# esw0116/DynaVSR

Hardware: AMD Instinct MI355X
Metric: inner-loop frames/sec/GPU (EDVR-M x4, 5x3x180x320): forward leg = BASELINE.json configs[1]; the inner MAML step and the per-frame pipeline are `inner_step` / `per_frame_pipeline` (higher is better)
Workload: dtype f32; 1 GPU; EDVR-M x4 forward (PCD deformable alignment + TSA fusion + reconstruction), clips of 1x5x3x180x320 -> 3x720x1280 (BASELINE.json configs[1]); one step = 2 clip(s) per GPU, one per HIP stream (adapt.super_resolve_video); clips_in_flight_per_gpu=2

## Files before the change

### dynavsr_amd/_lib.py

```python
import ctypes
import os
from ctypes import POINTER, Structure, c_char_p, c_float, c_int, c_longlong, c_size_t, c_void_p

import torch

_runtime = {"configured": False, "hw_queues": None, "effective": None}


def configure_runtime(hw_queues=6):
    if not _runtime["configured"]:
        user = os.environ.get("GPU_MAX_HW_QUEUES")
        late = torch.cuda.is_initialized()
        if user is None and not late:
            os.environ["GPU_MAX_HW_QUEUES"] = str(int(hw_queues))
        _runtime.update(configured=True, hw_queues=os.environ.get("GPU_MAX_HW_QUEUES"),
                        effective=(user is not None) or not late)
    return {"hw_queues": _runtime["hw_queues"], "effective": _runtime["effective"]}


def runtime_report(device=None):
    r = configure_runtime()
    overlaps = None
    if torch.cuda.is_available():
        with torch.cuda.device(device if device is not None else torch.cuda.current_device()):
# ... 81 lines not shown
        "dvsr_adam_step": (I, [POINTER(c_void_p)] * 4 + [POINTER(LL), I, F, F, F, F, F, I, P]),
        "dvsr_sgd_step": (I, [POINTER(c_void_p)] * 2 + [POINTER(LL), I, F, F, P]),
        "dvsr_replicate_tensors": (I, [POINTER(c_void_p)] * 2 + [POINTER(LL), I, I, P]),
        "dvsr_degrade_apply": (I, [P, P, P, I, I, I, I, I, I, I, I, I, P]),
        "dvsr_frame_metrics_workspace_bytes": (c_size_t, [I, I, I]),
        "dvsr_frame_metrics": (I, [P, P, I, I, I, F, F, P, P, P, c_size_t, P]),
        "dvsr_charbonnier_workspace_bytes": (c_size_t, []),
        "dvsr_charbonnier_forward": (I, [P, P, P, LL, F, P, c_size_t, P]),
        "dvsr_conv2d_packed_workspace_bytes": (c_size_t, [POINTER(Conv2dDesc)]),
        "dvsr_conv2d_forward_packed": (I, [POINTER(Conv2dDesc), P, c_size_t, P]),
        "dvsr_conv2d_dgrad_packed": (I, [POINTER(Conv2dDesc), P, P, P, c_size_t, P]),
        "dvsr_conv2d_packed_geometry": (I, [POINTER(Conv2dDesc), POINTER(ctypes.c_int * 4)]),
        "dvsr_conv2d_wgrad_geometry": (I, [POINTER(Conv2dDesc), I, I, POINTER(ctypes.c_int * 8)]),
        "dvsr_conv2d_wgrad_workspace_bytes": (c_size_t, [POINTER(Conv2dDesc), I]),
        "dvsr_conv2d_wgrad_bf16": (I, [POINTER(Conv2dDesc), P, P, P, P, c_size_t, P]),
        "dvsr_conv2d_wgrad_split3": (I, [POINTER(Conv2dDesc), P, P, P, P, c_size_t, P]),
        "dvsr_flow_warp_forward": (I, [P, P, P, I, I, I, I, LL, P]),
        "dvsr_flow_warp_backward": (I, [P, P, P, P, P, I, I, I, I, LL, P]),
        "dvsr_avgpool2_forward": (I, [P, P, LL, I, I, P]),
        "dvsr_avgpool2_backward": (I, [P, P, LL, I, I, I, P]),
        "dvsr_resize_bilinear_ac_forward": (I, [P, P, LL, I, I, I, I, F, LL, P]),
        "dvsr_resize_bilinear_ac_backward": (I, [P, P, LL, I, I, I, I, F, LL, P]),
        "dvsr_upsample_bicubic_ac_forward": (I, [P, P, LL, I, I, I, P]),
        "dvsr_upsample_bicubic_ac_backward": (I, [P, P, LL, I, I, I, P]),
        "dvsr_channel_affine": (I, [P, P, P, P, I, I, LL, LL, LL, I, P]),
        "dvsr_batchnorm_workspace_bytes": (c_size_t, [I]),
        "dvsr_batchnorm_forward": (I, [P] * 8 + [I, I, LL, I, F, F, I, P, c_size_t, P]),
        "dvsr_batchnorm_backward": (I, [P] * 9 + [I, I, LL, I, I, P, c_size_t, P]),
        "dvsr_temporal_gather3_forward": (I, [P, P, I, I, I, LL, I, P]),
        "dvsr_temporal_gather3_backward": (I, [P, P, I, I, I, LL, I, P]),
        "dvsr_dynamic_filter_forward": (I, [P, P, P, P, I, I, I, I, I, P]),
        "dvsr_dynamic_filter_backward": (I, [P, P, P, P, P, P, I, I, I, I, I, P]),
        "dvsr_conv3x3_small_cout": (I, [P, P, P, P, P, I, I, I, I, I, I, P]),
        "dvsr_conv1x1_dual": (I, [P, P, P, P, P, P, P, I, I, I, I, I, P]),
        "dvsr_patch_gather_forward": (I, [P, P, POINTER(c_int), POINTER(c_int), I, I, I, I, I, I, P]),
        "dvsr_patch_gather_backward": (I, [P, P, POINTER(c_int), POINTER(c_int), I, I, I, I, I, I, P]),
        "dvsr_l1_tail_forward": (I, [P, P, P, F, P, LL, P, c_size_t, P]),
        "dvsr_l1_tail_backward": (I, [P, P, P, F, P, LL, P]),
        "dvsr_charbonnier_backward": (I, [P, P, P, P, LL, F, P]),
        "dvsr_charbonnier_forward_grouped": (I, [P, P, P, LL, I, F, P, c_size_t, P]),
        "dvsr_charbonnier_backward_grouped": (I, [P, P, P, P, LL, I, F, P]),
        "dvsr_l1_tail_forward_grouped": (I, [P, P, P, F, P, LL, I, P, c_size_t, P]),
        "dvsr_l1_tail_backward_grouped": (I, [P, P, P, F, P, LL, I, P]),
        "dvsr_edvr_op_info": (I, [P, I, c_char_p, I, c_char_p, I, POINTER(ctypes.c_double),
                                  POINTER(ctypes.c_double)]),
        "dvsr_edvr_forward_timed": (I, [P, POINTER(c_void_p), P, P, P, c_size_t, P, POINTER(c_float)]),
        "dvsr_debug_mfma_peak": (LL, [P, I, I, I, I, P]),
        "dvsr_debug_mfma_shadow": (I, [P, P, I, I, I, I, I, P]),
        "dvsr_edvr_tensor_info": (I, [P, c_char_p, POINTER(LL), POINTER(LL)]),
        "dvsr_edvr_plan_work": (I, [P, POINTER(ctypes.c_double * 9)]),
        "dvsr_edvr_plan_work_nograd": (I, [P, POINTER(ctypes.c_double * 9)]),
        "dvsr_edvr_op_launch_count": (I, [P, I, I]),
        "dvsr_side_stream_overlaps": (I, [P]),
        "dvsr_edvr_op_output": (I, [P, I, I, POINTER(c_int), POINTER(LL), POINTER(LL)]),
        "dvsr_estimator_plan_work": (I, [P, POINTER(ctypes.c_double * 9)]),
        "dvsr_edvr_stream_create": (I, [POINTER(EdvrConfig), I, I, I, POINTER(c_void_p)]),
        "dvsr_edvr_stream_destroy": (None, [P]),
        "dvsr_edvr_stream_num_params": (I, [P]),
        "dvsr_edvr_stream_num_launches": (I, [P, I]),
        "dvsr_edvr_stream_cache_bytes": (c_size_t, [P]),
        "dvsr_edvr_stream_workspace_bytes": (c_size_t, [P]),
        "dvsr_edvr_stream_extract": (I, [P, POINTER(c_void_p), P, I, P, c_size_t, P, c_size_t, I, P]),
        "dvsr_edvr_stream_fuse": (I, [P, POINTER(c_void_p), POINTER(c_int), P, c_size_t, P, P, c_size_t, I, P]),
        "dvsr_frame_ingest": (I, [P, POINTER(FrameDesc), P, I, I, I, P]),
        "dvsr_frame_emit": (I, [P, I, I, P, POINTER(FrameDesc), F, F, P]),
        "dvsr_edvr_stream_extract_frame": (I, [P, POINTER(c_void_p), P, POINTER(FrameDesc), I, I, P, c_size_t, P, c_size_t, I,
# ... 42 lines not shown
```

### dynavsr_amd/csrc/conv_small.hip

```cpp
#include "common.h"
#include "kernels.h"

namespace dvsr {

struct SmallK {
  const float* x; const float* w; const float* bias; const float* res; float* y;
  int N, C, H, W, Cout, act, tiles_x, tiles_y, ntiles;
  int wdiv; long long w_gs; int b_gs;
};

typedef float f32x2 __attribute__((ext_vector_type(2)));

template <int COUT>
__global__ __launch_bounds__(256) void conv3x3_small_cout_kernel(SmallK a) {
  constexpr int CC = 8, TH = 8, TW = 64, IH = TH + 2, IW = TW + 2, PLANE = IH * IW, E = (PLANE + 255) / 256;
  constexpr int WPC = ((9 * COUT + 3) / 4) * 4;
  __shared__ __attribute__((aligned(16))) float s_in[2][CC * PLANE];
  extern __shared__ __attribute__((aligned(16))) float s_w[];
  const int tpx = (a.ntiles + 7) >> 3;
  const int tile = (blockIdx.x & 7) * tpx + (blockIdx.x >> 3);
  if ((int)(blockIdx.x >> 3) >= tpx || tile >= a.ntiles) return;
  const int tx_ = tile % a.tiles_x;
  const int t2 = tile / a.tiles_x;
  const int ty_ = t2 % a.tiles_y;
  const int n = t2 / a.tiles_y;
  const int oy0 = ty_ * TH, ox0 = tx_ * TW;
  const int tid = threadIdx.x;
  const int py = tid >> 5, px2 = (tid & 31) * 2;
  const size_t HW = (size_t)a.H * a.W;
  const float* xn = a.x + (size_t)n * a.C * HW;
  const float* wn = wset_ptr(a.w, a.w_gs, n, a.wdiv);
  const float* bn = wset_ptr(a.bias, a.b_gs, n, a.wdiv);

  unsigned eoff[E];
  bool evalid[E];
#pragma unroll
  for (int e = 0; e < E; ++e) {
    const int idx = tid + 256 * e;
    const int iy = idx / IW, ix = idx - iy * IW;
    const int gy = oy0 - 1 + iy, gx = ox0 - 1 + ix;
// ... 51 lines not shown
            const float wv = wq[wi >> 2][wi & 3];
            acc[o] = __builtin_elementwise_fma(f32x2{wv, wv}, f32x2{v[tx], v[tx + 1]}, acc[o]);
          }
      }
    }
  }
  const int oy = oy0 + py, ox = ox0 + px2;
  if (oy >= a.H || ox >= a.W) return;
  const bool two = ox + 1 < a.W;
  float bvs[COUT];
  f32x2 rvs[COUT];
#pragma unroll
  for (int o = 0; o < COUT; ++o) {
    bvs[o] = bn ? bn[o] : 0.f;
    const size_t idx = ((size_t)n * a.Cout + o) * HW + (size_t)oy * a.W + ox;
    rvs[o] = (a.res && two && (idx & 1) == 0) ? *reinterpret_cast<const f32x2*>(a.res + idx) : f32x2{0.f, 0.f};
  }
#pragma unroll
  for (int o = 0; o < COUT; ++o) {
    const float bv = bvs[o];
    f32x2 v = {apply_act(acc[o][0] + bv, a.act), apply_act(acc[o][1] + bv, a.act)};
    const size_t idx = ((size_t)n * a.Cout + o) * HW + (size_t)oy * a.W + ox;
    if (two && (idx & 1) == 0) {
      v += rvs[o];
      *reinterpret_cast<f32x2*>(a.y + idx) = v;
    } else {
      a.y[idx] = v[0] + (a.res ? a.res[idx] : 0.f);
      if (two) a.y[idx + 1] = v[1] + (a.res ? a.res[idx + 1] : 0.f);
    }
  }
}

struct SmallMfmaShape {
  static constexpr int TH = 6, TW = 56, RH = 8, RW = 64, X0 = 4, NPOS = RH * RW, APITCH = 68;
  static constexpr size_t LDS_BYTES = (size_t)(32 * APITCH + 27 * NPOS) * sizeof(float);
};

__device__ __forceinline__ __amdgpu_buffer_rsrc_t sm_rsrc(const float* base) {
  return __builtin_amdgcn_make_buffer_rsrc(const_cast<float*>(base), 0, 0x7fffffff, 0x00020000);
}
__device__ __forceinline__ f32x4 sm_load16(__amdgpu_buffer_rsrc_t rs, unsigned voff, unsigned soff) {
  return __builtin_bit_cast(f32x4, __builtin_amdgcn_raw_buffer_load_b128(rs, (int)voff, (int)soff, 0));
}

template <int COUT>
__global__ __launch_bounds__(256, 2) void conv3x3_small_cout_mfma_kernel(SmallK a) {
  using Sh = SmallMfmaShape;
  constexpr int TH = Sh::TH, TW = Sh::TW, RW = Sh::RW, NPOS = Sh::NPOS, AP = Sh::APITCH, NM = 9 * COUT;
  extern __shared__ __attribute__((aligned(16))) float s_mf[];
  float* const s_a = s_mf;
  float* const s_p = s_mf + 32 * AP;
  const int tpx = (a.ntiles + 7) >> 3;
  const int tile = (blockIdx.x & 7) * tpx + (blockIdx.x >> 3);
  if ((int)(blockIdx.x >> 3) >= tpx || tile >= a.ntiles) return;
  const int tx_ = tile % a.tiles_x;
  const int t2 = tile / a.tiles_x;
  const int ty_ = t2 % a.tiles_y;
  const int n = t2 / a.tiles_y;
  const int oy0 = ty_ * TH, ox0 = tx_ * TW;
  const int tid = threadIdx.x, lane = tid & 63;
  const int wave = __builtin_amdgcn_readfirstlane(tid >> 6);
  const int nn = lane & 31, kk = lane >> 5;
  const unsigned HW4 = (unsigned)a.H * a.W * 4u;
  const float* wn = wset_ptr(a.w, a.w_gs, n, a.wdiv);
  const float* bn = wset_ptr(a.bias, a.b_gs, n, a.wdiv);

  const int gy = oy0 - 1 + 2 * wave + (nn >> 4), gx = ox0 - Sh::X0 + 4 * (nn & 15);
  const bool inimg = (unsigned)gy < (unsigned)a.H && (unsigned)gx < (unsigned)a.W;
  const unsigned voff = inimg ? (unsigned)(8 * kk) * HW4 + (unsigned)(gy * a.W + gx) * 4u : 0x80000000u;
  const __amdgpu_buffer_rsrc_t xrs = sm_rsrc(a.x + (size_t)n * 64 * a.H * a.W);
  f32x4 B[2][16];
  auto issue = [&](int half) __attribute__((always_inline)) {
#pragma unroll
    for (int s = 0; s < 16; ++s) {
      const int c = 16 * (2 * half + (s >> 3)) + (s & 7);
      B[half][s] = sm_load16(xrs, voff, (unsigned)c * HW4);
    }
  };
  issue(0);
  for (int i = tid; i < 32 * 64; i += 256) {
    const int m = i >> 6, c = i & 63;
    const int tap = m / COUT, o = m - tap * COUT;
    s_a[m * AP + c] = m < NM ? wn[((size_t)o * 64 + c) * 9 + tap] : 0.f;
  }
  issue(1);
  __syncthreads();
  f32x4 A[8];
#pragma unroll
  for (int q = 0; q < 8; ++q) A[q] = *reinterpret_cast<const f32x4*>(s_a + nn * AP + 16 * (q >> 1) + 8 * kk + 4 * (q & 1));

  f32x16 acc[4];
#pragma unroll
  for (int j = 0; j < 4; ++j)
#pragma unroll
    for (int r = 0; r < 16; ++r) acc[j][r] = 0.f;
#pragma unroll
  for (int half = 0; half < 2; ++half)
#pragma unroll
    for (int s = 0; s < 16; ++s) {
      const int ch = 2 * half + (s >> 3), i = s & 7;
      const float av = A[2 * ch + (i >> 2)][i & 3];
#pragma unroll
      for (int j = 0; j < 4; ++j) acc[j] = __builtin_amdgcn_mfma_f32_32x32x2f32(av, B[half][s][j], acc[j], 0, 0, 0);
    }

#pragma unroll
  for (int r = 0; r < 16; ++r) {
    const int m = (r & 3) + 8 * (r >> 2) + 4 * kk;
    if (m < NM)
      *reinterpret_cast<f32x4*>(s_p + m * NPOS + 128 * wave + 4 * nn) = f32x4{acc[0][r], acc[1][r], acc[2][r], acc[3][r]};
  }
  __syncthreads();

  if (tid >= TH * (TW / 2)) return;
  const int y = tid / (TW / 2), xp = (tid - y * (TW / 2)) * 2;
  const int oy = oy0 + y, ox = ox0 + xp;
  if (oy >= a.H || ox >= a.W) return;
  float s0[COUT], s1[COUT];
#pragma unroll
  for (int o = 0; o < COUT; ++o) { s0[o] = 0.f; s1[o] = 0.f; }
#pragma unroll
  for (int dy = 0; dy < 3; ++dy) {
    const float* row = s_p + (y + dy) * RW + xp + Sh::X0 - 1;
#pragma unroll
    for (int dx = 0; dx < 3; ++dx)
#pragma unroll
      for (int o = 0; o < COUT; ++o) {
        const float* pm = row + ((dy * 3 + dx) * COUT + o) * NPOS + dx;
        s0[o] += pm[0];
        s1[o] += pm[1];
      }
  }
  const size_t HW = (size_t)a.H * a.W;
#pragma unroll
  for (int o = 0; o < COUT; ++o) {
    const float bv = bn ? bn[o] : 0.f;
    f32x2 v = {apply_act(s0[o] + bv, a.act), apply_act(s1[o] + bv, a.act)};
    const size_t idx = ((size_t)n * a.Cout + o) * HW + (size_t)oy * a.W + ox;
    if (a.res) v += *reinterpret_cast<const f32x2*>(a.res + idx);
    *reinterpret_cast<f32x2*>(a.y + idx) = v;
  }
}

template <int COUT>
static int launch_small_mfma(SmallK k, hipStream_t st) {
  using Sh = SmallMfmaShape;
  k.tiles_x = ceil_div(k.W, Sh::TW); k.tiles_y = ceil_div(k.H, Sh::TH); k.ntiles = k.tiles_x * k.tiles_y * k.N;
  auto kern = conv3x3_small_cout_mfma_kernel<COUT>;
  static PerDeviceOnce once;
  set_dyn_lds_once(once, (const void*)kern, Sh::LDS_BYTES);
  hipLaunchKernelGGL(kern, dim3(8 * ceil_div(k.ntiles, 8)), dim3(256), Sh::LDS_BYTES, st, k);
  return check_launch("conv3x3_small_cout_mfma_kernel");
}

int conv3x3_small_cout_run(const float* x, const float* w, const float* bias, const float* res, float* y, int N,
                           int C, int H, int W, int Cout, int act, hipStream_t st, int wdiv, long long w_gs, int b_gs) {
  DVSR_REQUIRE(x && w && y && Cout >= 1 && Cout <= 4, DVSR_ERR_INVALID, "conv3x3_small_cout: bad argument");
  SmallK k;
  k.x = x; k.w = w; k.bias = bias; k.res = res; k.y = y; k.N = N; k.C = C; k.H = H; k.W = W; k.Cout = Cout; k.act = act;
  k.wdiv = wdiv > 0 ? wdiv : 1; k.w_gs = w_gs; k.b_gs = b_gs;
  static const bool mfma_on = [] { const char* v = getenv("DVSR_CONV_LAST_MFMA"); return v && v[0] == '1'; }();
  if (mfma_on && C == 64 && Cout <= 3 && W % 4 == 0 && (unsigned long long)C * H * W * 4 < 0x7fffffffull &&
      ((((uintptr_t)x | (uintptr_t)y | (uintptr_t)res) & 15) == 0) && w_gs % 4 == 0) {
    if (Cout == 1) return launch_small_mfma<1>(k, st);
    if (Cout == 2) return launch_small_mfma<2>(k, st);
    return launch_small_mfma<3>(k, st);
  }
  k.tiles_x = ceil_div(W, 64); k.tiles_y = ceil_div(H, 8); k.ntiles = k.tiles_x * k.tiles_y * N;
  auto wbytes = [&](int cout) { return (size_t)ceil_div(C, 8) * 8 * (((9 * cout + 3) / 4) * 4) * sizeof(float); };
  switch (Cout) {
    case 1: hipLaunchKernelGGL(conv3x3_small_cout_kernel<1>, dim3(8 * ceil_div(k.ntiles, 8)), dim3(256), wbytes(1), st, k); break;
    case 2: hipLaunchKernelGGL(conv3x3_small_cout_kernel<2>, dim3(8 * ceil_div(k.ntiles, 8)), dim3(256), wbytes(2), st, k); break;
    case 3: hipLaunchKernelGGL(conv3x3_small_cout_kernel<3>, dim3(8 * ceil_div(k.ntiles, 8)), dim3(256), wbytes(3), st, k); break;
    default: hipLaunchKernelGGL(conv3x3_small_cout_kernel<4>, dim3(8 * ceil_div(k.ntiles, 8)), dim3(256), wbytes(4), st, k); break;
  }
  return check_launch("conv3x3_small_cout_kernel");
}

}

extern "C" int dvsr_conv3x3_small_cout(const float* x, const float* w, const float* bias, const float* res, float* y, int N,
                                       int C, int H, int W, int Cout, int act, dvsr_stream_t stream) {
  DVSR_REQUIRE(N > 0 && C > 0 && H > 0 && W > 0, DVSR_ERR_INVALID, "conv3x3_small_cout: empty tensor");
  return dvsr::conv3x3_small_cout_run(x, w, bias, res, y, N, C, H, W, Cout, act, (hipStream_t)stream, 1, 0, 0);
}
```

### dynavsr_amd/csrc/engine.hip

```cpp
#include <algorithm>
#include <cstdlib>
#include <string>
#include <vector>

#include "common.h"
#include "kernels.h"
#include "small_grid.h"

namespace dvsr {

enum { SP_ARENA = 0, SP_INPUT = 1, SP_OUTPUT = 2, SP_NONE = 3 };
struct T {
  int space = SP_NONE;
  size_t off = 0, numel = 0;
  bool valid() const { return space != SP_NONE; }
};

enum OpType { OP_CONV, OP_DCN, OP_UP, OP_POOL, OP_GATE, OP_BLEND, OP_ADD, OP_PAD, OP_MEANSUB, OP_ADDMEAN };

struct Op {
  OpType type;
  const char* name = "";
  T x0, x1, res, y, y2;
  int pw = -1, pb = -1;
// ... 830 lines not shown

static int run_forward_op(const dvsr_edvr_plan& p, const Op& o, const float* const* P, const Bases& bs, hipStream_t st) {
  switch (o.type) {
    case OP_CONV: {
      dvsr_conv2d_desc d = {};
      d.x0 = bs.at(o.x0); d.x1 = bs.at(o.x1); d.w = P[o.pw]; d.bias = P[o.pb]; d.res = bs.at(o.res);
      d.y = bs.at(o.y);
      d.N = o.N; d.c0 = o.c0; d.c1 = o.c1; d.H = o.H; d.W = o.W; d.Cout = o.Cout; d.ks = o.ks;
      d.stride = o.stride; d.pad = conv_pad(o); d.act = o.act; d.pixel_shuffle = o.ps;
      if (o.pad_out) { d.y = bs.at(o.ypad); d.pixel_shuffle = o.pad_out; }
      if (!p.use_v1 && (o.dual >= 0 || o.fused_into >= 0)) {
        const Op& oa = o.dual >= 0 ? o : p.ops[o.fused_into];
        const Op& ob = p.ops[oa.dual];
        const long long HW = (long long)oa.H * oa.W;
        auto plain1x1 = [](const Op& q) {
          return q.type == OP_CONV && q.ks == 1 && q.stride == 1 && q.c1 == 0 && q.Cout == 64 && !q.res.valid() && !q.ps && !q.wmap && !q.pad_out;
        };
        const bool pair_ok = plain1x1(oa) && plain1x1(ob) && oa.act == ob.act && oa.c0 == ob.c0 && oa.N == ob.N && oa.H == ob.H &&
                             oa.W == ob.W && oa.x0.space == ob.x0.space && oa.x0.off == ob.x0.off;
        if (pair_ok && conv1x1_dual_ok(bs.at(oa.x0), P[oa.pw], P[ob.pw], bs.at(oa.y), bs.at(ob.y), oa.c0, HW)) {
          if (o.fused_into >= 0) return DVSR_OK;
          return conv1x1_dual_run(bs.at(oa.x0), P[oa.pw], P[oa.pb], P[ob.pw], P[ob.pb], bs.at(oa.y), bs.at(ob.y), oa.N, oa.c0,
                                  (int)HW, oa.act, st, p.wsets > 1 ? oa.N / p.wsets : 1,
                                  p.wsets > 1 ? (long long)oa.Cout * oa.c0 : 0, p.wsets > 1 ? oa.Cout : 0);
        }
      }
      if (o.wmap) d.w = bs.arena + o.w2_off;
      d.x1_bdiv = o.x1_bdiv; d.x0_bstride = o.x0_bs; d.x1_bstride = o.x1_bs;
      if (p.use_v1) return conv2d_run(d, ConvExtra(), st);
      if (o.Cout <= 4 && o.ks == 3 && o.stride == 1 && !o.c1 && !o.ps && !o.x0_bs && o.pad < 0)
        return conv3x3_small_cout_run(d.x0, d.w, d.bias, d.res, d.y, o.N, o.c0, o.H, o.W, o.Cout, o.act, st,
                                      p.wsets > 1 ? o.N / p.wsets : 1, p.wsets > 1 ? (long long)o.Cout * o.c0 * 9 : 0,
                                      p.wsets > 1 ? o.Cout : 0);
      for (const Op::Launch& l : o.launches[bs.mode]) {
        ConvExtra ex;
        set_wsets(p, o.N, l.pack.floats, o.Cout, &ex);
        int rc = conv2d_packed_run(launch_desc(d, o, l.role, bs.at(o.pre)), bs.arena + l.pack.off, ex, l.pack.geo, st);
        if (rc != DVSR_OK) return rc;
      }
      return DVSR_OK;
    }
    case OP_DCN: {
      const float* om = bs.at(o.x1);
      const long long bstride = (long long)o.dg * 27 * o.H * o.W;
      if (!p.use_v1 && o.dcn_pack.floats)
        return mdcn_forward_packed_run(bs.at(o.x0), om, bstride, om + (size_t)o.dg * 18 * o.H * o.W, bstride, 1,
                                       bs.arena + o.dcn_pack.off, P[o.pb], bs.at(o.y), o.N, o.c0, o.H, o.W, o.Cout,
                                       o.dg, o.act, st, p.wsets > 1 ? o.N / p.wsets : 1,
                                       p.wsets > 1 ? (long long)o.dcn_pack.floats : 0, p.wsets > 1 ? o.Cout : 0, mdcn_pack_layout(o.W));
      return mdcn_forward_run(bs.at(o.x0), om, bstride, om + (size_t)o.dg * 18 * o.H * o.W, bstride, 1,
                              P[o.pw], P[o.pb], bs.at(o.y), o.N, o.c0, o.H, o.W, o.Cout, 3, 3, 1, 1,
                              1, 1, o.dg, o.act, st);
    }
    case OP_UP:
      return upsample_bilinear_fwd(bs.at(o.x0), bs.at(o.y), o.planes, o.H, o.W, o.S, o.mul, st);
    case OP_POOL:
      return pool3s2_fwd(bs.at(o.x0), bs.at(o.y), bs.at(o.y2), o.planes, o.H, o.W, st);
    case OP_GATE:
      return tsa_gate_fwd(bs.at(o.x0), bs.at(o.x1), bs.at(o.res), bs.at(o.y), bs.at(o.y2), o.gB, o.gN,
                          o.gC, o.gHW, st);
    case OP_BLEND:
      return tsa_blend_fwd(bs.at(o.x0), bs.at(o.x1), bs.at(o.res), bs.at(o.y), o.y.numel, st);
    case OP_PAD:
      if (o.fused_into >= 0) return DVSR_OK;
      return pad_fwd(bs.at(o.x0), bs.at(o.y), o.pmode, o.N, o.c0, o.H, o.W, o.T, st);
    case OP_MEANSUB:
// ... 683 lines not shown
```

### dynavsr_amd/csrc/kernels.h

```cpp
#pragma once
#include "../../include/dynavsr_hip.h"
#include "common.h"

namespace dvsr {

struct ConvExtra {
  int wt = 0;
  int w_ctot = 0, w_coff = 0;
  int in_ps = 0;
  int in_dil = 0, Hs = 0, Ws = 0;
  int accum = 0;
  const float* gmask = nullptr;
  int gmask_act = 0;
  int wdiv = 1; long long w_gs = 0; int b_gs = 0;
};
int conv2d_run(const dvsr_conv2d_desc& d, const ConvExtra& ex, hipStream_t st);

int mdcn_forward_run(const float* x, const float* off, long long off_bs, const float* msk,
                     long long msk_bs, int mask_logit, const float* w, const float* b, float* out,
                     int N, int C, int H, int W, int Cout, int kh, int kw, int stride, int pad,
                     int dil, int groups, int dg, int act, hipStream_t st);

enum class ConvKernel : int {
  REG = 0,
// ... 38 lines not shown
  ALLOW_NONE = 0,
  ALLOW_KSPLIT = 1,
  ALLOW_DMA_HALO = 2,
  ALLOW_WINO = 4,
  ALLOW_WINO_F4 = 8,
  ALLOW_SHARED_DEVICE = 16,
  ALLOW_ONLY_F4 = 32,
};
constexpr ConvAllow operator|(ConvAllow a, ConvAllow b) { return static_cast<ConvAllow>(static_cast<int>(a) | static_cast<int>(b)); }
constexpr ConvAllow without(ConvAllow a, ConvAllow b) { return static_cast<ConvAllow>(static_cast<int>(a) & ~static_cast<int>(b)); }
ConvGeo conv2_choose(int ks, int stride, int N, int Ho, int Wo, int Cout, int Ctot, ConvAllow allow = ALLOW_KSPLIT);
size_t conv2_pack_floats(int ks, int Cout, int Ctot, int cc, int bf, PackLayout layout);
PackEntry conv2_pack_entry(const float* w, float* P, int ks, int Cout, int Ctot, int cc, int bf, PackLayout layout, int wt = 0,
                           int w_ctot = 0, int w_coff = 0);
inline size_t conv2_pack_floats(int ks, int Cout, int Ctot, const ConvGeo& g) {
  return conv2_pack_floats(ks, Cout, Ctot, g.cc, g.bf, pack_layout(g.kernel));
}
inline PackEntry conv2_pack_entry(const float* w, float* P, int ks, int Cout, int Ctot, const ConvGeo& g, int wt = 0, int w_ctot = 0,
                                  int w_coff = 0) {
  return conv2_pack_entry(w, P, ks, Cout, Ctot, g.cc, g.bf, pack_layout(g.kernel), wt, w_ctot, w_coff);
}
double conv2_f4_occupied_cycles(int N, int Ho, int Wo, int Cout, int Ctot, int th);
int pack_weights_wino_run(const PackTable& t, hipStream_t st);
int pack_weights_wino3_run(const PackTable& t, hipStream_t st);
int pack_weights_wino5_run(const PackTable& t, hipStream_t st);
int conv2d_packed_run(const dvsr_conv2d_desc& d, const float* wp, const ConvExtra& ex, const ConvGeo& geo,
                      hipStream_t st);

bool conv1x1_dual_ok(const float* x, const float* w0, const float* w1, const float* y0, const float* y1, int Cin, long long HW);
int conv1x1_dual_run(const float* x, const float* w0, const float* b0, const float* w1, const float* b1, float* y0, float* y1,
                     int N, int Cin, int HW, int act, hipStream_t st, int wdiv = 1, long long w_gs = 0, int b_gs = 0);
int conv3x3_small_cout_run(const float* x, const float* w, const float* bias, const float* res, float* y, int N,
                           int C, int H, int W, int Cout, int act, hipStream_t st, int wdiv = 1, long long w_gs = 0,
                           int b_gs = 0);

struct WgradReduceEntry {
  float* partial; float* dbp; float* dW; float* db;
  int nslot, KK, OP, CP, Cout, Cin, Ctot, c_off;
  int ngroups = 1;
  long long dW_gs = 0, db_gs = 0;
};
constexpr int WGRAD_REDUCE_BATCH = 44;
struct WgradReduceTable {
  int n;
  WgradReduceEntry e[WGRAD_REDUCE_BATCH];
};
int wgrad_reduce_batch(const WgradReduceEntry* entries, int n, hipStream_t st, int blocks = 96);
struct WgradDesc {
  const float* x = nullptr; long long x_bs = 0; int x_bdiv = 1;
  const float* gy = nullptr; int gy_ps = 0;
  float* dW = nullptr; float* db = nullptr;
  int N = 0, Cin = 0, H = 0, W = 0, Cout = 0, Ctot = 0, c_off = 0, ks = 0, stride = 1, pad = -1;
  int groups = 1; long long dW_gs = 0, db_gs = 0;
  int mode = 0;
};
enum class WgradKernel : int {
  SIMPLE = 0,
  PIPE = 1,
  BF16 = 2,
  SPLIT_SCALAR = 3,
  SPLIT_VECTOR = 4,
  SPLIT_WAVE8 = 5,
};
constexpr bool on_bf16_pipe(WgradKernel k) { return k >= WgradKernel::BF16; }
constexpr bool on_bf16_split(WgradKernel k) { return k >= WgradKernel::SPLIT_SCALAR; }
struct WgradGeo {
  WgradKernel kernel = WgradKernel::PIPE;
// ... 113 lines not shown
```

### include/dynavsr_hip.h

```cpp
#ifndef DYNAVSR_HIP_H_
#define DYNAVSR_HIP_H_

#include <stddef.h>

#ifdef __cplusplus
extern "C" {
#endif

#define DVSR_OK 0
#define DVSR_ERR_INVALID (-1)
#define DVSR_ERR_UNSUPPORTED (-2)
#define DVSR_ERR_WORKSPACE (-3)
#define DVSR_ERR_HIP (-4)

#define DVSR_ACT_NONE 0
#define DVSR_ACT_LRELU 1
#define DVSR_ACT_RELU 2

typedef void* dvsr_stream_t;

const char* dvsr_last_error(void);
int dvsr_version(void);

int dvsr_mdcn_forward(const float* x, const float* offset, const float* mask, const float* w,
// ... 204 lines not shown
                           dvsr_stream_t stream);
int dvsr_resize_bilinear_ac_forward(const float* x, float* y, long long planes, int H, int W, int Ho, int Wo, float mul,
                                    long long y_plane_stride, dvsr_stream_t stream);
int dvsr_resize_bilinear_ac_backward(const float* grad_y, float* grad_x, long long planes, int H, int W, int Ho, int Wo,
                                     float mul, long long gy_plane_stride, dvsr_stream_t stream);
int dvsr_upsample_bicubic_ac_forward(const float* x, float* y, long long planes, int H, int W, int scale,
                                     dvsr_stream_t stream);
int dvsr_upsample_bicubic_ac_backward(const float* grad_y, float* grad_x, long long planes, int H, int W, int scale,
                                      dvsr_stream_t stream);
int dvsr_channel_affine(const float* x, const float* scale, const float* shift, float* out, int N, int C, long long HW,
                        long long x_bstride, long long out_bstride, int accumulate, dvsr_stream_t stream);
size_t dvsr_batchnorm_workspace_bytes(int C);
int dvsr_batchnorm_forward(const float* x, const float* gamma, const float* beta, float* running_mean,
                           float* running_var, float* y, float* save_mean, float* save_rstd, int N, int C, long long HW,
                           int training, float momentum, float eps, int relu, void* workspace, size_t workspace_bytes,
                           dvsr_stream_t stream);
int dvsr_batchnorm_backward(const float* x, const float* grad_y, const float* y, const float* gamma,
                            const float* save_mean, const float* save_rstd, float* grad_x, float* grad_gamma,
                            float* grad_beta, int N, int C, long long HW, int training, int relu, void* workspace,
                            size_t workspace_bytes, dvsr_stream_t stream);

int dvsr_temporal_gather3_forward(const float* x, float* y, int B, int T, int C, long long HW, int pad_t,
                                  dvsr_stream_t stream);
int dvsr_temporal_gather3_backward(const float* grad_y, float* grad_x, int B, int T, int C, long long HW, int pad_t,
                                   dvsr_stream_t stream);
int dvsr_dynamic_filter_forward(const float* x_center, const float* filter_logits, const float* residual, float* out,
                                int B, int H, int W, int scale, int adapt_official, dvsr_stream_t stream);
int dvsr_dynamic_filter_backward(const float* x_center, const float* filter_logits, const float* grad_out,
                                 float* grad_logits, float* grad_residual, float* grad_x_center, int B, int H, int W,
                                 int scale, int adapt_official, dvsr_stream_t stream);

int dvsr_conv3x3_small_cout(const float* x, const float* w, const float* bias, const float* res, float* y, int N, int C, int H,
                            int W, int Cout, int act, dvsr_stream_t stream);

int dvsr_conv1x1_dual(const float* x, const float* w0, const float* b0, const float* w1, const float* b1, float* y0, float* y1,
                      int N, int Cin, int H, int W, int act, dvsr_stream_t stream);

int dvsr_patch_gather_forward(const float* src, float* dst, const int* py, const int* px, int P, int planes, int H, int W,
                              int edge, int scale, dvsr_stream_t stream);
int dvsr_patch_gather_backward(const float* grad_dst, float* grad_src, const int* py, const int* px, int P, int planes,
                               int H, int W, int edge, int scale, dvsr_stream_t stream);

int dvsr_adam_step(float* const* params, const float* const* grads, float* const* exp_avg,
                   float* const* exp_avg_sq, const long long* numel, int n_tensors, float lr, float beta1,
                   float beta2, float eps, float weight_decay, int step, dvsr_stream_t stream);
int dvsr_sgd_step(float* const* params, const float* const* grads, const long long* numel, int n_tensors,
                  float lr, float weight_decay, dvsr_stream_t stream);
int dvsr_replicate_tensors(const float* const* src, float* const* dst, const long long* numel, int n_tensors, int copies,
                           dvsr_stream_t stream);

size_t dvsr_frame_metrics_workspace_bytes(int C, int H, int W);
int dvsr_frame_metrics(const float* sr, const float* gt, int C, int H, int W, float lo, float hi,
                       unsigned char* sr_hwc_u8, double* out, void* workspace, size_t workspace_bytes,
                       dvsr_stream_t stream);

int dvsr_degrade_apply(const float* img, const float* kernels, float* out, int N, int C, int H, int W, int K,
                       int scale, int n_kernels, int kernel_offset, int quantise, dvsr_stream_t stream);

#ifdef __cplusplus
}
#endif
#endif
```

Measured before the change: 262.1 frames/s.

## Add MFMA small-Cin first conv and row-streaming small-Cout MFMA conv, enable by default

```diff
diff --git a/dynavsr_amd/_lib.py b/dynavsr_amd/_lib.py
--- a/dynavsr_amd/_lib.py
+++ b/dynavsr_amd/_lib.py
@@ -137,6 +137,8 @@
         "dvsr_dynamic_filter_forward": (I, [P, P, P, P, I, I, I, I, I, P]),
         "dvsr_dynamic_filter_backward": (I, [P, P, P, P, P, P, I, I, I, I, I, P]),
         "dvsr_conv3x3_small_cout": (I, [P, P, P, P, P, I, I, I, I, I, I, P]),
+        "dvsr_conv3x3_small_cout_sets": (I, [P, P, P, P, P, I, I, I, I, I, I, I, I, P]),
+        "dvsr_conv3x3_small_cin": (I, [P, LL, P, P, P, I, I, I, I, I, I, I, P]),
         "dvsr_conv1x1_dual": (I, [P, P, P, P, P, P, P, I, I, I, I, I, P]),
         "dvsr_patch_gather_forward": (I, [P, P, POINTER(c_int), POINTER(c_int), I, I, I, I, I, I, P]),
         "dvsr_patch_gather_backward": (I, [P, P, POINTER(c_int), POINTER(c_int), I, I, I, I, I, I, P]),
diff --git a/dynavsr_amd/csrc/conv_small.hip b/dynavsr_amd/csrc/conv_small.hip
--- a/dynavsr_amd/csrc/conv_small.hip
+++ b/dynavsr_amd/csrc/conv_small.hip
@@ -6,6 +6,7 @@
 struct SmallK {
   const float* x; const float* w; const float* bias; const float* res; float* y;
   int N, C, H, W, Cout, act, tiles_x, tiles_y, ntiles;
+  int seg_steps;
   int wdiv; long long w_gs; int b_gs;
 };
 
@@ -123,8 +124,9 @@
 }
 
 struct SmallMfmaShape {
-  static constexpr int TH = 6, TW = 56, RH = 8, RW = 64, X0 = 4, NPOS = RH * RW, APITCH = 68;
-  static constexpr size_t LDS_BYTES = (size_t)(32 * APITCH + 27 * NPOS) * sizeof(float);
+  static constexpr int TW = 56, RW = 64, X0 = 4, SH = 8, RING = SH + 2, PP = RING * RW, APITCH = 68, MAX_STEPS = 12;
+  static constexpr size_t LDS_BYTES = (size_t)(27 * PP) * sizeof(float);
+  static_assert(32 * APITCH <= 9 * PP, "the weight image must fit under the P planes of COUT = 1");
 };
 
 __device__ __forceinline__ __amdgpu_buffer_rsrc_t sm_rsrc(const float* base) {
@@ -137,10 +139,10 @@
 template <int COUT>
 __global__ __launch_bounds__(256, 2) void conv3x3_small_cout_mfma_kernel(SmallK a) {
   using Sh = SmallMfmaShape;
-  constexpr int TH = Sh::TH, TW = Sh::TW, RW = Sh::RW, NPOS = Sh::NPOS, AP = Sh::APITCH, NM = 9 * COUT;
+  constexpr int TW = Sh::TW, RW = Sh::RW, SH = Sh::SH, RING = Sh::RING, PP = Sh::PP, AP = Sh::APITCH, NM = 9 * COUT;
   extern __shared__ __attribute__((aligned(16))) float s_mf[];
   float* const s_a = s_mf;
-  float* const s_p = s_mf + 32 * AP;
+  float* const s_p = s_mf;
   const int tpx = (a.ntiles + 7) >> 3;
   const int tile = (blockIdx.x & 7) * tpx + (blockIdx.x >> 3);
   if ((int)(blockIdx.x >> 3) >= tpx || tile >= a.ntiles) return;
@@ -148,7 +150,10 @@
   const int t2 = tile / a.tiles_x;
   const int ty_ = t2 % a.tiles_y;
   const int n = t2 / a.tiles_y;
-  const int oy0 = ty_ * TH, ox0 = tx_ * TW;
+  const int seg = SH * a.seg_steps - 2;
+  const int oy0 = ty_ * seg, ox0 = tx_ * TW;
+  const int oy_end = min(a.H, oy0 + seg);
+  const int nsteps = (oy_end - oy0 + 2 + SH - 1) / SH;
   const int tid = threadIdx.x, lane = tid & 63;
   const int wave = __builtin_amdgcn_readfirstlane(tid >> 6);
   const int nn = lane & 31, kk = lane >> 5;
@@ -156,87 +161,125 @@
   const float* wn = wset_ptr(a.w, a.w_gs, n, a.wdiv);
   const float* bn = wset_ptr(a.bias, a.b_gs, n, a.wdiv);
 
-  const int gy = oy0 - 1 + 2 * wave + (nn >> 4), gx = ox0 - Sh::X0 + 4 * (nn & 15);
-  const bool inimg = (unsigned)gy < (unsigned)a.H && (unsigned)gx < (unsigned)a.W;
-  const unsigned voff = inimg ? (unsigned)(8 * kk) * HW4 + (unsigned)(gy * a.W + gx) * 4u : 0x80000000u;
+  const int hr = 2 * wave + (nn >> 4), gx = ox0 - Sh::X0 + 4 * (nn & 15);
+  auto offset_of = [&](int k) __attribute__((always_inline)) {
+    const int gy = oy0 - 1 + SH * k + hr;
+    const bool inimg = k < nsteps && (unsigned)gy < (unsigned)a.H && (unsigned)gx < (unsigned)a.W;
+    return inimg ? (unsigned)(8 * kk) * HW4 + (unsigned)(gy * a.W + gx) * 4u : 0x80000000u;
+  };
   const __amdgpu_buffer_rsrc_t xrs = sm_rsrc(a.x + (size_t)n * 64 * a.H * a.W);
   f32x4 B[2][16];
-  auto issue = [&](int half) __attribute__((always_inline)) {
+  auto issue = [&](int half, unsigned voff) __attribute__((always_inline)) {
 #pragma unroll
     for (int s = 0; s < 16; ++s) {
       const int c = 16 * (2 * half + (s >> 3)) + (s & 7);
       B[half][s] = sm_load16(xrs, voff, (unsigned)c * HW4);
     }
   };
-  issue(0);
-  for (int i = tid; i < 32 * 64; i += 256) {
-    const int m = i >> 6, c = i & 63;
+  const unsigned voff0 = offset_of(0);
+  issue(0, voff0);
+  float wv[8];
+#pragma unroll
+  for (int e = 0; e < 8; ++e) {
+    const int m = min((tid + 256 * e) >> 6, NM - 1), c = tid & 63;
     const int tap = m / COUT, o = m - tap * COUT;
-    s_a[m * AP + c] = m < NM ? wn[((size_t)o * 64 + c) * 9 + tap] : 0.f;
-  }
-  issue(1);
+    wv[e] = wn[((size_t)o * 64 + c) * 9 + tap];
+  }
+#pragma unroll
+  for (int e = 0; e < 8; ++e) {
+    const int m = (tid + 256 * e) >> 6, c = tid & 63;
+    s_a[m * AP + c] = m < NM ? wv[e] : 0.f;
+  }
+  issue(1, voff0);
   __syncthreads();
   f32x4 A[8];
 #pragma unroll
   for (int q = 0; q < 8; ++q) A[q] = *reinterpret_cast<const f32x4*>(s_a + nn * AP + 16 * (q >> 1) + 8 * kk + 4 * (q & 1));
 
-  f32x16 acc[4];
-#pragma unroll
-  for (int j = 0; j < 4; ++j)
-#pragma unroll
-    for (int r = 0; r < 16; ++r) acc[j][r] = 0.f;
-#pragma unroll
-  for (int half = 0; half < 2; ++half)
-#pragma unroll
-    for (int s = 0; s < 16; ++s) {
-      const int ch = 2 * half + (s >> 3), i = s & 7;
-      const float av = A[2 * ch + (i >> 2)][i & 3];
-#pragma unroll
-      for (int j = 0; j < 4; ++j) acc[j] = __builtin_amdgcn_mfma_f32_32x32x2f32(av, B[half][s][j], acc[j], 0, 0, 0);
-    }
-
-#pragma unroll
-  for (int r = 0; r < 16; ++r) {
-    const int m = (r & 3) + 8 * (r >> 2) + 4 * kk;
-    if (m < NM)
-      *reinterpret_cast<f32x4*>(s_p + m * NPOS + 128 * wave + 4 * nn) = f32x4{acc[0][r], acc[1][r], acc[2][r], acc[3][r]};
-  }
-  __syncthreads();
-
-  if (tid >= TH * (TW / 2)) return;
   const int y = tid / (TW / 2), xp = (tid - y * (TW / 2)) * 2;
-  const int oy = oy0 + y, ox = ox0 + xp;
-  if (oy >= a.H || ox >= a.W) return;
-  float s0[COUT], s1[COUT];
-#pragma unroll
-  for (int o = 0; o < COUT; ++o) { s0[o] = 0.f; s1[o] = 0.f; }
-#pragma unroll
-  for (int dy = 0; dy < 3; ++dy) {
-    const float* row = s_p + (y + dy) * RW + xp + Sh::X0 - 1;
-#pragma unroll
-    for (int dx = 0; dx < 3; ++dx)
+  const int ox = ox0 + xp;
+  const size_t HW = (size_t)a.H * a.W;
+  const __amdgpu_buffer_rsrc_t rrs =
+      __builtin_amdgcn_make_buffer_rsrc(const_cast<float*>(a.res ? a.res + (size_t)n * a.Cout * HW : nullptr), 0,
+                                        a.res ? 0x7fffffff : 0, 0x00020000);
+  float bv[COUT];
+#pragma unroll
+  for (int o = 0; o < COUT; ++o) bv[o] = bn ? bn[o] : 0.f;
+
+  for (int k = 0; k < nsteps; ++k) {
+    const unsigned vnext = offset_of(k + 1);
+    const int r0 = k ? SH * k - 2 : 0, rc = k ? SH : SH - 2;
+    const int oy = oy0 + r0 + y;
+    const bool out = y < rc && oy < oy_end && ox < a.W;
+    const unsigned ooff = out ? (unsigned)(oy * a.W + ox) * 4u : 0x80000000u;
+    f32x2 rv[COUT];
+#pragma unroll
+    for (int o = 0; o < COUT; ++o)
+      rv[o] = __builtin_bit_cast(f32x2, __builtin_amdgcn_raw_buffer_load_b64(rrs, (int)ooff, (int)((unsigned)o * HW4), 0));
+    f32x16 acc[4];
+#pragma unroll
+    for (int j = 0; j < 4; ++j)
+#pragma unroll
+      for (int r = 0; r < 16; ++r) acc[j][r] = 0.f;
+#pragma unroll
+    for (int half = 0; half < 2; ++half) {
+#pragma unroll
+      for (int s = 0; s < 16; ++s) {
+        const int ch = 2 * half + (s >> 3), i = s & 7;
+        const float av = A[2 * ch + (i >> 2)][i & 3];
+#pragma unroll
+        for (int j = 0; j < 4; ++j) acc[j] = __builtin_amdgcn_mfma_f32_32x32x2f32(av, B[half][s][j], acc[j], 0, 0, 0);
+      }
+      __builtin_amdgcn_sched_barrier(0);
+      issue(half, vnext);
+      __builtin_amdgcn_sched_barrier(0);
+    }
+
+    __syncthreads();
+    float* const pw = s_p + ((SH * k + hr) % RING) * RW + 4 * (nn & 15);
+#pragma unroll
+    for (int r = 0; r < 16; ++r) {
+      const int m = (r & 3) + 8 * (r >> 2) + 4 * kk;
+      if (m < NM) *reinterpret_cast<f32x4*>(pw + m * PP) = f32x4{acc[0][r], acc[1][r], acc[2][r], acc[3][r]};
+    }
+    __syncthreads();
+
+    if (out) {
+      float s0[COUT], s1[COUT];
+#pragma unroll
+      for (int o = 0; o < COUT; ++o) { s0[o] = 0.f; s1[o] = 0.f; }
+#pragma unroll
+      for (int dy = 0; dy < 3; ++dy) {
+        const float* row = s_p + ((r0 + y + dy) % RING) * RW + xp + Sh::X0 - 1;
+#pragma unroll
+        for (int dx = 0; dx < 3; ++dx)
+#pragma unroll
+          for (int o = 0; o < COUT; ++o) {
+            const float* pm = row + ((dy * 3 + dx) * COUT + o) * PP + dx;
+            s0[o] += pm[0];
+            s1[o] += pm[1];
+          }
+      }
 #pragma unroll
       for (int o = 0; o < COUT; ++o) {
-        const float* pm = row + ((dy * 3 + dx) * COUT + o) * NPOS + dx;
-        s0[o] += pm[0];
-        s1[o] += pm[1];
-      }
-  }
-  const size_t HW = (size_t)a.H * a.W;
-#pragma unroll
-  for (int o = 0; o < COUT; ++o) {
-    const float bv = bn ? bn[o] : 0.f;
-    f32x2 v = {apply_act(s0[o] + bv, a.act), apply_act(s1[o] + bv, a.act)};
-    const size_t idx = ((size_t)n * a.Cout + o) * HW + (size_t)oy * a.W + ox;
-    if (a.res) v += *reinterpret_cast<const f32x2*>(a.res + idx);
-    *reinterpret_cast<f32x2*>(a.y + idx) = v;
+        f32x2 v = {apply_act(s0[o] + bv[o], a.act), apply_act(s1[o] + bv[o], a.act)};
+        v += rv[o];
+        *reinterpret_cast<f32x2*>(a.y + ((size_t)n * a.Cout + o) * HW + (size_t)oy * a.W + ox) = v;
+      }
+    }
   }
 }
 
 template <int COUT>
-static int launch_small_mfma(SmallK k, hipStream_t st) {
+static int launch_small_mfma(SmallK k, int seg_steps, hipStream_t st) {
   using Sh = SmallMfmaShape;
-  k.tiles_x = ceil_div(k.W, Sh::TW); k.tiles_y = ceil_div(k.H, Sh::TH); k.ntiles = k.tiles_x * k.tiles_y * k.N;
+  k.tiles_x = ceil_div(k.W, Sh::TW);
+  const long long resident = 2ll * device_cus();
+  int steps = 1;
+  while (steps < Sh::MAX_STEPS && (long long)k.tiles_x * ceil_div(k.H, Sh::SH * steps - 2) * k.N > resident) ++steps;
+  if (seg_steps > 0) steps = seg_steps;
+  k.seg_steps = steps;
+  k.tiles_y = ceil_div(k.H, Sh::SH * steps - 2); k.ntiles = k.tiles_x * k.tiles_y * k.N;
   auto kern = conv3x3_small_cout_mfma_kernel<COUT>;
   static PerDeviceOnce once;
   set_dyn_lds_once(once, (const void*)kern, Sh::LDS_BYTES);
@@ -245,17 +288,19 @@
 }
 
 int conv3x3_small_cout_run(const float* x, const float* w, const float* bias, const float* res, float* y, int N,
-                           int C, int H, int W, int Cout, int act, hipStream_t st, int wdiv, long long w_gs, int b_gs) {
+                           int C, int H, int W, int Cout, int act, hipStream_t st, int wdiv, long long w_gs, int b_gs,
+                           int seg_steps) {
   DVSR_REQUIRE(x && w && y && Cout >= 1 && Cout <= 4, DVSR_ERR_INVALID, "conv3x3_small_cout: bad argument");
+  DVSR_REQUIRE(seg_steps >= 0 && seg_steps <= 4096, DVSR_ERR_INVALID, "conv3x3_small_cout: seg_steps out of range");
   SmallK k;
   k.x = x; k.w = w; k.bias = bias; k.res = res; k.y = y; k.N = N; k.C = C; k.H = H; k.W = W; k.Cout = Cout; k.act = act;
   k.wdiv = wdiv > 0 ? wdiv : 1; k.w_gs = w_gs; k.b_gs = b_gs;
-  static const bool mfma_on = [] { const char* v = getenv("DVSR_CONV_LAST_MFMA"); return v && v[0] == '1'; }();
+  static const bool mfma_on = [] { const char* v = getenv("DVSR_CONV_LAST_MFMA"); return !(v && v[0] == '0'); }();
   if (mfma_on && C == 64 && Cout <= 3 && W % 4 == 0 && (unsigned long long)C * H * W * 4 < 0x7fffffffull &&
       ((((uintptr_t)x | (uintptr_t)y | (uintptr_t)res) & 15) == 0) && w_gs % 4 == 0) {
-    if (Cout == 1) return launch_small_mfma<1>(k, st);
-    if (Cout == 2) return launch_small_mfma<2>(k, st);
-    return launch_small_mfma<3>(k, st);
+    if (Cout == 1) return launch_small_mfma<1>(k, seg_steps, st);
+    if (Cout == 2) return launch_small_mfma<2>(k, seg_steps, st);
+    return launch_small_mfma<3>(k, seg_steps, st);
   }
   k.tiles_x = ceil_div(W, 64); k.tiles_y = ceil_div(H, 8); k.ntiles = k.tiles_x * k.tiles_y * N;
   auto wbytes = [&](int cout) { return (size_t)ceil_div(C, 8) * 8 * (((9 * cout + 3) / 4) * 4) * sizeof(float); };
@@ -275,3 +320,13 @@
   DVSR_REQUIRE(N > 0 && C > 0 && H > 0 && W > 0, DVSR_ERR_INVALID, "conv3x3_small_cout: empty tensor");
   return dvsr::conv3x3_small_cout_run(x, w, bias, res, y, N, C, H, W, Cout, act, (hipStream_t)stream, 1, 0, 0);
 }
+
+extern "C" int dvsr_conv3x3_small_cout_sets(const float* x, const float* w, const float* bias, const float* res, float* y, int N,
+                                            int C, int H, int W, int Cout, int act, int wsets, int seg_steps,
+                                            dvsr_stream_t stream) {
+  DVSR_REQUIRE(N > 0 && C > 0 && H > 0 && W > 0, DVSR_ERR_INVALID, "conv3x3_small_cout_sets: empty tensor");
+  DVSR_REQUIRE(wsets >= 1 && N % wsets == 0, DVSR_ERR_INVALID, "conv3x3_small_cout_sets: N must be a multiple of wsets");
+  const bool sets = wsets > 1;
+  return dvsr::conv3x3_small_cout_run(x, w, bias, res, y, N, C, H, W, Cout, act, (hipStream_t)stream, sets ? N / wsets : 1,
+                                      sets ? (long long)Cout * C * 9 : 0, sets ? Cout : 0, seg_steps);
+}
diff --git a/dynavsr_amd/csrc/conv_small_cin.hip b/dynavsr_amd/csrc/conv_small_cin.hip
--- /dev/null
+++ b/dynavsr_amd/csrc/conv_small_cin.hip
@@ -0,0 +1,194 @@
+#include "common.h"
+#include "kernels.h"
+
+namespace dvsr {
+
+struct SmallCinK {
+  const float* x; const float* w; const float* bias; float* y;
+  int N, H, W, act, tiles_x, tiles_y, ntiles, seg_steps;
+  long long x_bs;
+  int wdiv; long long w_gs; int b_gs;
+};
+
+struct SmallCinShape {
+  static constexpr int TW = 64, SH = 8, IW = TW + 2, RING = 2 * SH + 2, PITCH = 68, MAX_STEPS = 16;
+  static constexpr int WGS_PER_CU = 3;
+};
+
+template <int CIN>
+__global__ __launch_bounds__(256, 2) void conv3x3_small_cin_kernel(SmallCinK a) {
+  using Sh = SmallCinShape;
+  constexpr int TW = Sh::TW, SH = Sh::SH, IW = Sh::IW, RING = Sh::RING, PITCH = Sh::PITCH, CP = RING * PITCH;
+  constexpr int K = 9 * CIN, KS = (K + 1) / 2;
+  constexpr int NLD = ((SH + 2) * IW + 255) / 256;
+  __shared__ float s_x[CIN * CP];
+  __shared__ float s_b[64];
+  const int tile = blockIdx.x;
+  const int tx_ = tile % a.tiles_x;
+  const int t2 = tile / a.tiles_x;
+  const int ty_ = t2 % a.tiles_y;
+  const int n = t2 / a.tiles_y;
+  const int seg = SH * a.seg_steps;
+  const int oy0 = ty_ * seg, ox0 = tx_ * TW;
+  const int oy_end = min(a.H, oy0 + seg);
+  const int nsteps = (oy_end - oy0 + SH - 1) / SH;
+  const int tid = threadIdx.x, lane = tid & 63;
+  const int wave = __builtin_amdgcn_readfirstlane(tid >> 6);
+  const int nn = lane & 31, kk = lane >> 5;
+  const unsigned HW4 = (unsigned)a.H * a.W * 4u;
+  const size_t HW = (size_t)a.H * a.W;
+  const float* wn = wset_ptr(a.w, a.w_gs, n, a.wdiv);
+  const float* bn = wset_ptr(a.bias, a.b_gs, n, a.wdiv);
+
+  float A[2][KS];
+#pragma unroll
+  for (int mb = 0; mb < 2; ++mb)
+#pragma unroll
+    for (int s = 0; s < KS; ++s) A[mb][s] = wn[(size_t)(32 * mb + nn) * K + min(2 * s + kk, K - 1)];
+  if (2 * KS > K) {
+#pragma unroll
+    for (int mb = 0; mb < 2; ++mb) A[mb][KS - 1] = kk ? 0.f : A[mb][KS - 1];
+  }
+  if (tid < 64) s_b[tid] = bn ? bn[tid] : 0.f;
+
+  const __amdgpu_buffer_rsrc_t xrs = __builtin_amdgcn_make_buffer_rsrc(
+      const_cast<float*>(a.x + (size_t)n * a.x_bs), 0, (int)((unsigned)CIN * HW4), 0x00020000);
+  const __amdgpu_buffer_rsrc_t yrs =
+      __builtin_amdgcn_make_buffer_rsrc(a.y + (size_t)n * 64 * HW, 0, (int)(64u * HW4), 0x00020000);
+  const float slope = a.act == ACT_LRELU ? 0.1f : 1.f;
+  const bool relu = a.act == ACT_RELU;
+  auto act_of = [&](float v) __attribute__((always_inline)) { return v > 0.f ? v : (relu ? 0.f : slope * v); };
+  float rin[CIN][NLD];
+  auto fetch = [&](int h0, int nrows) __attribute__((always_inline)) {
+#pragma unroll
+    for (int i = 0; i < NLD; ++i) {
+      const int idx = tid + 256 * i;
+      const int row = idx / IW, col = idx - row * IW;
+      const int gy = oy0 - 1 + h0 + row, gx = ox0 - 1 + col;
+      const bool ok = row < nrows && (unsigned)gy < (unsigned)a.H && (unsigned)gx < (unsigned)a.W;
+      const unsigned off = ok ? (unsigned)(gy * a.W + gx) * 4u : 0x80000000u;
+#pragma unroll
+      for (int c = 0; c < CIN; ++c)
+        rin[c][i] = __builtin_bit_cast(float, __builtin_amdgcn_raw_buffer_load_b32(xrs, (int)off, (int)((unsigned)c * HW4), 0));
+    }
+  };
+  auto stash = [&](int h0, int nrows) __attribute__((always_inline)) {
+#pragma unroll
+    for (int i = 0; i < NLD; ++i) {
+      const int idx = tid + 256 * i;
+      const int row = idx / IW, col = idx - row * IW;
+      if (row < nrows) {
+#pragma unroll
+        for (int c = 0; c < CIN; ++c) s_x[c * CP + ((h0 + row) % RING) * PITCH + col] = rin[c][i];
+      }
+    }
+  };
+  fetch(0, SH + 2);
+  stash(0, SH + 2);
+
+  const int prow = 2 * wave + (nn >> 4), pcol = 4 * (nn & 15);
+  const int ox = ox0 + pcol;
+  for (int k = 0; k < nsteps; ++k) {
+    __syncthreads();
+    const int nxt = k + 1 < nsteps ? SH : 0;
+    fetch(SH * (k + 1) + 2, nxt);
+    int rs[3];
+#pragma unroll
+    for (int dy = 0; dy < 3; ++dy) rs[dy] = ((SH * k + prow + dy) % RING) * PITCH + pcol;
+    const int oy = oy0 + SH * k + prow;
+    const bool out = oy < oy_end && ox < a.W;
+    const unsigned yoff = out ? (unsigned)(4 * kk) * HW4 + (unsigned)(oy * a.W + ox) * 4u : 0x80000000u;
+#pragma unroll
+    for (int mb = 0; mb < 2; ++mb) {
+      __builtin_amdgcn_sched_barrier(0);
+      f32x16 acc[4];
+#pragma unroll
+      for (int j = 0; j < 4; ++j)
+#pragma unroll
+        for (int r = 0; r < 16; ++r) acc[j][r] = 0.f;
+#pragma unroll
+      for (int s = 0; s < KS; ++s) {
+        const int k0 = 2 * s, k1 = 2 * s + 1 < K ? 2 * s + 1 : K - 1;
+        const int a0 = (k0 / 9) * CP + rs[(k0 % 9) / 3] + k0 % 3, a1 = (k1 / 9) * CP + rs[(k1 % 9) / 3] + k1 % 3;
+        const float* src = s_x + (kk ? a1 : a0);
+        float b[4];
+#pragma unroll
+        for (int j = 0; j < 4; ++j) b[j] = src[j];
+        if (2 * s + 1 >= K) {
+#pragma unroll
+          for (int j = 0; j < 4; ++j) b[j] = kk ? 0.f : b[j];
+        }
+#pragma unroll
+        for (int j = 0; j < 4; ++j) acc[j] = __builtin_amdgcn_mfma_f32_32x32x2f32(A[mb][s], b[j], acc[j], 0, 0, 0);
+      }
+#pragma unroll
+      for (int r = 0; r < 16; ++r) {
+        const int co = 32 * mb + (r & 3) + 8 * (r >> 2);
+        const float b0 = s_b[co + 4 * kk];
+        const f32x4 v = {act_of(acc[0][r] + b0), act_of(acc[1][r] + b0), act_of(acc[2][r] + b0), act_of(acc[3][r] + b0)};
+        __builtin_amdgcn_raw_buffer_store_b128(__builtin_bit_cast(__attribute__((ext_vector_type(4))) unsigned, v), yrs, (int)yoff,
+                                               (int)((unsigned)co * HW4), 0);
+      }
+    }
+    stash(SH * (k + 1) + 2, nxt);
+  }
+}
+
+template <int CIN>
+static int launch_small_cin(SmallCinK k, int seg_steps, hipStream_t st) {
+  using Sh = SmallCinShape;
+  k.tiles_x = ceil_div(k.W, Sh::TW);
+  const long long resident = (long long)Sh::WGS_PER_CU * device_cus();
+  int steps = 1;
+  while (steps < Sh::MAX_STEPS && (long long)k.tiles_x * ceil_div(k.H, Sh::SH * steps) * k.N > resident) ++steps;
+  if (seg_steps > 0) steps = seg_steps;
+  k.seg_steps = steps;
+  k.tiles_y = ceil_div(k.H, Sh::SH * steps); k.ntiles = k.tiles_x * k.tiles_y * k.N;
+  hipLaunchKernelGGL(conv3x3_small_cin_kernel<CIN>, dim3(k.ntiles), dim3(256), 0, st, k);
+  return check_launch("conv3x3_small_cin_kernel");
+}
+
+bool conv3x3_small_cin_ok(const float* y, int Cin, int H, int W) {
+  return Cin >= 1 && Cin <= 4 && W % 4 == 0 && ((uintptr_t)y & 15) == 0 && (unsigned long long)64 * H * W * 4 < 0x7fffffffull;
+}
+
+int conv3x3_small_cin_run(const float* x, long long x_bs, const float* w, const float* bias, float* y, int N, int Cin, int H,
+                          int W, int act, hipStream_t st, int wdiv, long long w_gs, int b_gs, int seg_steps) {
+  DVSR_REQUIRE(x && w && y, DVSR_ERR_INVALID, "conv3x3_small_cin: null pointer");
+  DVSR_REQUIRE(conv3x3_small_cin_ok(y, Cin, H, W), DVSR_ERR_UNSUPPORTED, "conv3x3_small_cin: Cin=%d W=%d / alignment", Cin, W);
+  DVSR_REQUIRE(seg_steps >= 0 && seg_steps <= 4096, DVSR_ERR_INVALID, "conv3x3_small_cin: seg_steps out of range");
+  SmallCinK k;
+  k.x = x; k.w = w; k.bias = bias; k.y = y; k.N = N; k.H = H; k.W = W; k.act = act;
+  k.x_bs = x_bs ? x_bs : (long long)Cin * H * W;
+  k.wdiv = wdiv > 0 ? wdiv : 1; k.w_gs = w_gs; k.b_gs = b_gs;
+  switch (Cin) {
+    case 1: return launch_small_cin<1>(k, seg_steps, st);
+    case 2: return launch_small_cin<2>(k, seg_steps, st);
+    case 3: return launch_small_cin<3>(k, seg_steps, st);
+    default: return launch_small_cin<4>(k, seg_steps, st);
+  }
+}
+
+}
+
+extern "C" int dvsr_conv3x3_small_cin(const float* x, long long x_bstride, const float* w, const float* bias, float* y, int N,
+                                      int Cin, int H, int W, int act, int wsets, int seg_steps, dvsr_stream_t stream) {
+  DVSR_REQUIRE(N > 0 && Cin > 0 && H > 0 && W > 0, DVSR_ERR_INVALID, "conv3x3_small_cin: empty tensor");
+  DVSR_REQUIRE(wsets >= 1 && N % wsets == 0, DVSR_ERR_INVALID, "conv3x3_small_cin: N must be a multiple of wsets");
+  const bool sets = wsets > 1;
+  const int wdiv = N / wsets;
+  if (dvsr::conv3x3_small_cin_ok(y, Cin, H, W))
+    return dvsr::conv3x3_small_cin_run(x, x_bstride, w, bias, y, N, Cin, H, W, act, (hipStream_t)stream, sets ? wdiv : 1,
+                                       sets ? (long long)64 * Cin * 9 : 0, sets ? 64 : 0, seg_steps);
+  const long long xs = x_bstride ? x_bstride : (long long)Cin * H * W;
+  for (int g = 0; g < wsets; ++g) {
+    dvsr_conv2d_desc d = {};
+    d.x0 = x + (size_t)g * wdiv * xs; d.w = w + (size_t)g * 64 * Cin * 9; d.bias = bias ? bias + (size_t)g * 64 : nullptr;
+    d.y = y + (size_t)g * wdiv * 64 * H * W;
+    d.N = sets ? wdiv : N; d.c0 = Cin; d.H = H; d.W = W; d.Cout = 64; d.ks = 3; d.stride = 1; d.pad = 1;
+    d.act = act; d.x1_bdiv = 1; d.x0_bstride = x_bstride;
+    const int rc = dvsr::conv2d_run(d, dvsr::ConvExtra(), (hipStream_t)stream);
+    if (rc != DVSR_OK) return rc;
+  }
+  return DVSR_OK;
+}
diff --git a/dynavsr_amd/csrc/engine.hip b/dynavsr_amd/csrc/engine.hip
--- a/dynavsr_amd/csrc/engine.hip
+++ b/dynavsr_amd/csrc/engine.hip
@@ -886,6 +886,11 @@
         return conv3x3_small_cout_run(d.x0, d.w, d.bias, d.res, d.y, o.N, o.c0, o.H, o.W, o.Cout, o.act, st,
                                       p.wsets > 1 ? o.N / p.wsets : 1, p.wsets > 1 ? (long long)o.Cout * o.c0 * 9 : 0,
                                       p.wsets > 1 ? o.Cout : 0);
+      if (o.c0 <= 4 && o.Cout == 64 && o.ks == 3 && o.stride == 1 && !o.c1 && !o.ps && !o.pad_out && !o.wmap && o.pad < 0 &&
+          !o.res.valid() && conv3x3_small_cin_ok(d.y, o.c0, o.H, o.W))
+        return conv3x3_small_cin_run(d.x0, o.x0_bs, d.w, d.bias, d.y, o.N, o.c0, o.H, o.W, o.act, st,
+                                     p.wsets > 1 ? o.N / p.wsets : 1, p.wsets > 1 ? (long long)o.Cout * o.c0 * 9 : 0,
+                                     p.wsets > 1 ? o.Cout : 0);
       for (const Op::Launch& l : o.launches[bs.mode]) {
         ConvExtra ex;
         set_wsets(p, o.N, l.pack.floats, o.Cout, &ex);
diff --git a/dynavsr_amd/csrc/kernels.h b/dynavsr_amd/csrc/kernels.h
--- a/dynavsr_amd/csrc/kernels.h
+++ b/dynavsr_amd/csrc/kernels.h
@@ -94,7 +94,10 @@
                      int N, int Cin, int HW, int act, hipStream_t st, int wdiv = 1, long long w_gs = 0, int b_gs = 0);
 int conv3x3_small_cout_run(const float* x, const float* w, const float* bias, const float* res, float* y, int N,
                            int C, int H, int W, int Cout, int act, hipStream_t st, int wdiv = 1, long long w_gs = 0,
-                           int b_gs = 0);
+                           int b_gs = 0, int seg_steps = 0);
+bool conv3x3_small_cin_ok(const float* y, int Cin, int H, int W);
+int conv3x3_small_cin_run(const float* x, long long x_bs, const float* w, const float* bias, float* y, int N, int Cin, int H,
+                          int W, int act, hipStream_t st, int wdiv = 1, long long w_gs = 0, int b_gs = 0, int seg_steps = 0);
 
 struct WgradReduceEntry {
   float* partial; float* dbp; float* dW; float* db;
diff --git a/include/dynavsr_hip.h b/include/dynavsr_hip.h
--- a/include/dynavsr_hip.h
+++ b/include/dynavsr_hip.h
@@ -260,6 +260,11 @@
 
 int dvsr_conv3x3_small_cout(const float* x, const float* w, const float* bias, const float* res, float* y, int N, int C, int H,
                             int W, int Cout, int act, dvsr_stream_t stream);
+int dvsr_conv3x3_small_cout_sets(const float* x, const float* w, const float* bias, const float* res, float* y, int N, int C,
+                                 int H, int W, int Cout, int act, int wsets, int seg_steps, dvsr_stream_t stream);
+
+int dvsr_conv3x3_small_cin(const float* x, long long x_bstride, const float* w, const float* bias, float* y, int N, int Cin,
+                           int H, int W, int act, int wsets, int seg_steps, dvsr_stream_t stream);
 
 int dvsr_conv1x1_dual(const float* x, const float* w0, const float* b0, const float* w1, const float* b1, float* y0, float* y1,
                       int N, int Cin, int H, int W, int act, dvsr_stream_t stream);
```

Result: no change. 264.1 frames/s (median of 6 runs) (+0.7%).
